# cgbur/llama2.zig

Measured on AMD Instinct MI355X. Metric: tokens/s (argmax, -t 0), higher is better.
Workload: dtype f32; 1 GPU; llama2-7b shape, fp32 llama2.c-v0 checkpoint (dim 4096, hidden 11008, L 32, H 32, kv 32, V 32000, S 2048), greedy from BOS, seeded synthetic weights; parallelism=1 GPU

## Files before the change

### llama2.zig_amd/binding.py

```python
from __future__ import annotations

import ctypes as C
import os
import re

import numpy as np

_HERE = os.path.dirname(os.path.abspath(__file__))
PRODUCT_LIB_PATH = os.path.join(_HERE, "libllama2_hip.so")
LIB_PATH = os.environ.get("L2Z_LIB") or os.path.join(_HERE, "libllama2_hip_test.so")
HEADER_PATH = os.path.join(os.path.dirname(_HERE), "include", "llama2_hip.h")
TEST_HEADER_PATH = os.path.join(os.path.dirname(_HERE), "include", "llama2_hip_test.h")

OK, ERR_INVALID, ERR_NO_DEVICE, ERR_HIP, ERR_OOM, ERR_COMM, ERR_STATE = 0, -1, -2, -3, -4, -5, -6
COMM_ID_BYTES = 128
COMM_IPC_BYTES = 64
KINDS = ["qkv", "attn", "wo", "ffn13", "ffn2", "cls", "argmax", "gather"]


class L2ZError(RuntimeError):
    def __init__(self, code: int, msg: str):
        super().__init__(f"llama2_hip error {code}: {msg}")
        self.code = code

# ... 1277 lines not shown


def softmax(x) -> np.ndarray:
    o = np.array(x, np.float32, copy=True)
    _chk(lib().l2z_softmax(_fp(o), o.size))
    return o


def vector_dot_product(x, y) -> np.float32:
    x, y = _f32(x), _f32(y)
    o = np.zeros(1, np.float32)
    _chk(lib().l2z_vector_dot_product(_fp(o), _fp(x), _fp(y), x.size))
    return o[0]


def vector_weighted_sum_rows(xout_len: int, rows, row_stride: int, weights) -> np.ndarray:
    rows, weights = _f32(rows), _f32(weights)
    o = np.empty(xout_len, np.float32)
    _chk(lib().l2z_vector_weighted_sum_rows(_fp(o), xout_len, _fp(rows), rows.size, row_stride,
                                            _fp(weights), weights.size))
    return o


ATTN_FORMS = {"auto": 0, "fast256": 1, "fast1024": 2, "split": 3, "generic": 4}


def attention_decode(q, kcache, vcache, pos: int, n_heads: int, n_kv_heads: int, head_size: int,
                     seq_len: int, form: str = "auto", nch: int = 0) -> np.ndarray:
    q, kcache, vcache = _f32(q), _f32(kcache), _f32(vcache)
    assert q.size == n_heads * head_size and kcache.size == seq_len * n_kv_heads * head_size
    out = np.empty(n_heads * head_size, np.float32)
    _chk(lib().l2z_attention_decode(ATTN_FORMS[form], nch, _fp(out), _fp(q), _fp(kcache), _fp(vcache),
                                    pos, n_heads, n_kv_heads, head_size, seq_len))
    return out


def q8_quantize(x, gs: int):
    x = _f32(x).reshape(-1)
    q = np.empty(x.size, np.int8)
    s = np.empty(x.size // gs, np.float32)
    _chk(lib().l2z_q8_quantize(_fp(x), x.size, gs, q.ctypes.data_as(C.POINTER(C.c_int8)), _fp(s)))
    return q, s


def q8_matmul(xq, xs, wq, ws, gs: int) -> np.ndarray:
    wq = np.ascontiguousarray(wq, dtype=np.int8)
    d, n = wq.shape
# ... 105 lines not shown
```

### llama2.zig_amd/csrc/attention.hip

```cpp
#include "kernel_common.h"

namespace l2z {
namespace {

constexpr int kAttnUB = 4;

template <bool VEC>
__device__ __forceinline__ void attn_scores(const float *qs, const float *__restrict__ kbase,
                                            int kv_stride, int head_size, int T, float div,
                                            float *att)
{
    const AttnGeom ge = attn_geom(head_size, VEC);
    const int g = threadIdx.x / ge.TPR, c0 = threadIdx.x % ge.TPR;
    for (int t0 = g; t0 < T; t0 += ge.G * kAttnUB) {
        float p[kAttnUB];
#pragma unroll
        for (int i = 0; i < kAttnUB; i++) p[i] = 0.0f;
        for (int c = c0; c < ge.E; c += ge.TPR) {
            if (VEC) {
                v4f kv[kAttnUB];
#pragma unroll
                for (int i = 0; i < kAttnUB; i++) {
                    int t = t0 + ge.G * i;
                    t = t < T ? t : T - 1;
// ... 64 lines not shown
            for (int t0 = g; t0 < T; t0 += ge.G * kAttnUB) {
                float vv[kAttnUB], w[kAttnUB];
#pragma unroll
                for (int i = 0; i < kAttnUB; i++) {
                    const int t = t0 + ge.G * i;
                    const int tc = t < T ? t : T - 1;
                    vv[i] = vbase[(size_t)tc * (size_t)kv_stride + c];
                    w[i] = t < T ? att[tc] : 0.0f;
                }
#pragma unroll
                for (int i = 0; i < kAttnUB; i++) acc = fmaf(vv[i], w[i], acc);
            }
            part[(size_t)g * head_size + c] = acc;
        }
    }
    __syncthreads();
    for (int i = threadIdx.x; i < head_size; i += blockDim.x) {
        float s = part[i];
        for (int gg = 1; gg < ge.G; gg++) s += part[(size_t)gg * head_size + i];
        out[i] = s;
    }
}

template <bool WT = false>
__device__ __forceinline__ void reduce_partials(const float *part, int G, int hs, float *out,
                                                const P2pArgs *push = nullptr, int push_e = 0,
                                                size_t push_idx0 = 0)
{
    int R = 1;
    while (R * 2 <= G && R * 2 * hs <= (int)blockDim.x && R < 16) R <<= 1;
    const int i = threadIdx.x / R, r = threadIdx.x % R;
    float s = 0.0f;
    if (i < hs)
        for (int gg = r; gg < G; gg += R) s += part[(size_t)gg * hs + i];
    s = lanes_sum(s, R);
    if (i < hs && r == 0) {
        if constexpr (WT) {
            __hip_atomic_store(out + i, s, __ATOMIC_RELAXED, __HIP_MEMORY_SCOPE_AGENT);
        } else {
            out[i] = s;
            if (push) p2p_ll_push(push, push_e, push_idx0 + (size_t)i, s);
        }
    }
}

constexpr int kFastUB = 8;
constexpr int kAttnFastBlock = 1024;

struct AttnLane {
    int g, c0, cc, G, TPR;
    size_t stride;
};

template <bool NT>
__device__ __forceinline__ void attn_load_round(const float *base, const AttnLane &ln, int t0, int bound, v4f (&r)[kFastUB])
{
#pragma unroll
    for (int i = 0; i < kFastUB; i++) {
        int t = t0 + ln.G * i;
        t = t < bound ? t : bound - 1;
        const v4f *p = (const v4f *)(base + (size_t)t * ln.stride) + ln.cc;
        if constexpr (NT) r[i] = ldg_nt(p);
        else r[i] = *p;
    }
}

template <bool NT>
__device__ __forceinline__ void attn_score_rounds(const float *kbase, const AttnLane &ln, v4f qv, v4f (&kr)[kFastUB], int T,
                                                  float div, float *att)
{
    const v4f zero = {0.f, 0.f, 0.f, 0.f};
    for (int t0 = ln.g;;) {
#pragma unroll
        for (int i = 0; i < kFastUB; i++) {
            float p = hsum4(fma4(qv, kr[i], zero));
            p = lanes_sum(p, ln.TPR);
            const int t = t0 + ln.G * i;
            if (ln.c0 == 0 && t < T) att[t] = p / div;
        }
        t0 += ln.G * kFastUB;
        if (t0 >= T) break;
        attn_load_round<NT>(kbase, ln, t0, T, kr);
    }
}

template <bool NT>
__device__ __forceinline__ v4f attn_wsum_rounds(const float *vbase, const AttnLane &ln, v4f (&vr)[kFastUB], int T, const float *w_)
{
    v4f acc = {0.f, 0.f, 0.f, 0.f};
    for (int t0 = ln.g;;) {
#pragma unroll
        for (int i = 0; i < kFastUB; i++) {
            const int t = t0 + ln.G * i;
            const float w = t < T ? w_[t] : 0.0f;
            acc.x = fmaf(vr[i].x, w, acc.x);
            acc.y = fmaf(vr[i].y, w, acc.y);
            acc.z = fmaf(vr[i].z, w, acc.z);
            acc.w = fmaf(vr[i].w, w, acc.w);
        }
        t0 += ln.G * kFastUB;
        if (t0 >= T) break;
        attn_load_round<NT>(vbase, ln, t0, T, vr);
    }
    return acc;
}

__device__ __forceinline__ AttnLane attn_lane(const AttnGeom &ge, size_t stride)
{
    AttnLane ln;
    ln.g = threadIdx.x / ge.TPR;
    ln.c0 = threadIdx.x % ge.TPR;
    ln.cc = ln.c0 < ge.E ? ln.c0 : 0;
    ln.G = ge.G;
    ln.TPR = ge.TPR;
    ln.stride = stride;
    return ln;
}

template <int NT, bool SPEC>
__global__ __launch_bounds__(NT) void attention_fast_kernel(const AttnArgs a)
{
    extern __shared__ __attribute__((aligned(16))) float lds[];
// ... 5 lines not shown
    const int h = blockIdx.x;
    const int kvh = h / a.kv_mul;
    const float *kbase = a.kcache + (size_t)kvh * a.kv_head;
    const float *vbase = a.vcache + (size_t)kvh * a.kv_head;
    const AttnLane ln = attn_lane(ge, (size_t)a.kv_row);
    const bool active = ln.c0 < ge.E;
    const v4f zero = {0.f, 0.f, 0.f, 0.f};

    const int T = *a.pos_ptr + 1;
    const int lim = SPEC ? a.seq_len : T;
    const v4f qv = active ? ((const v4f *)(a.q + (size_t)h * hs))[ln.cc] : zero;
    v4f kr[kFastUB], vr[kFastUB];
    attn_load_round<false>(kbase, ln, ln.g, lim, kr);
    attn_load_round<false>(vbase, ln, ln.g, lim, vr);
    attn_score_rounds<false>(kbase, ln, qv, kr, T, sqrtf((float)hs), att);
    __syncthreads();
    wave_softmax(att, prob, T);
    const v4f acc = attn_wsum_rounds<false>(vbase, ln, vr, T, prob);
    if (active) ((v4f *)(part + (size_t)ln.g * hs))[ln.cc] = acc;
    __syncthreads();
    reduce_partials(part, ge.G, hs, a.xb + (size_t)h * hs, a.push,
                    a.push ? a.push_ctl[kCtlEpoch] + a.push_gi : 0,
                    a.push ? (size_t)a.push->rank * a.push->count + (size_t)h * hs : 0);
}

__host__ __device__ inline int attn_split_per(int T, int nch) { return (((T + nch - 1) / nch) + 1) & ~1; }

__device__ __forceinline__ void combine_chunks(const float *p, int nch, int hs, float *xb_h,
                                               const P2pArgs *push, int push_e, size_t push_idx0)
{
    constexpr int kMaxCh = 16;
    float mc[kMaxCh], lc[kMaxCh];
#pragma unroll
    for (int c = 0; c < kMaxCh; c++) {
        const int cc = c < nch ? c : 0;
        mc[c] = p[(size_t)cc * (hs + 4) + hs];
        lc[c] = p[(size_t)cc * (hs + 4) + hs + 1];
    }
    float M = -INFINITY;
#pragma unroll
    for (int c = 0; c < kMaxCh; c++)
        if (c < nch) M = fmaxf(M, mc[c]);
    float den = 0.0f;
#pragma unroll
    for (int c = 0; c < kMaxCh; c++) {
        mc[c] = c < nch ? expf(mc[c] - M) : 0.0f;
// ... 203 lines not shown
static bool attn_vec_shape(const AttnArgs &a)
{
    return (a.head_size % 4) == 0 && (a.kv_row % 4) == 0 && (a.kv_head % 4) == 0 && aligned16(a.q) && aligned16(a.kcache) &&
           aligned16(a.vcache);
}
static bool attn_fast_shape(const AttnArgs &a) { return attn_vec_shape(a) && a.head_size <= 256; }

bool attention_push_supported(const AttnArgs &a) { return attn_fast_shape(a); }

bool attention_split_supported(const AttnArgs &a) { return attn_fast_shape(a); }

hipError_t launch_attention_split(const AttnArgs &a, int n_heads_local, int nch, float *part,
                                  int *arrivals, hipStream_t st, bool small)
{
    const int nt = small ? kBlock : kAttnFastBlock;
    const AttnGeom ge = attn_geom(a.head_size, true, nt);
    const int max_local = attn_split_per(a.seq_len, nch);
    const size_t lds = (size_t)(2 * ((max_local + 3) & ~3) + ge.G * a.head_size) * sizeof(float);
    const dim3 grid(n_heads_local * nch);
    return small ? launch_lds(attention_split_kernel<kBlock>, grid, dim3(kBlock), lds, st, a, nch, part, arrivals)
                 : launch_lds(attention_split_kernel<kAttnFastBlock>, grid, dim3(kAttnFastBlock), lds, st, a, nch, part, arrivals);
}

hipError_t launch_attention(const AttnArgs &a, int n_heads_local, hipStream_t st, int form)
{
    const bool vec = attn_vec_shape(a);
    const dim3 grid(n_heads_local);
    if (attn_fast_shape(a) && form != 4) {
        const int forced = form == 1 ? kBlock : form == 2 ? kAttnFastBlock : 0;
        const int nt = forced ? forced : (a.seq_len > 512 ? kAttnFastBlock : kBlock);
        const AttnGeom gf = attn_geom(a.head_size, true, nt);
        const size_t lds_fast = (size_t)(2 * ((a.seq_len + 3) & ~3) + gf.G * a.head_size) * sizeof(float);
        return nt == kAttnFastBlock ? launch_lds(attention_fast_kernel<kAttnFastBlock, false>, grid, dim3(kAttnFastBlock), lds_fast, st, a)
                                    : launch_lds(attention_fast_kernel<kBlock, true>, grid, dim3(kBlock), lds_fast, st, a);
    }
    const size_t lds = attention_lds_bytes(a.head_size, a.seq_len, vec);
    return vec ? launch_lds(attention_kernel<true>, grid, dim3(kBlock), lds, st, a)
               : launch_lds(attention_kernel<false>, grid, dim3(kBlock), lds, st, a);
}

hipError_t launch_dot(float *out, const float *x, const float *y, int n, hipStream_t st)
{
    const bool vec = (n % 4) == 0 && aligned16(x) && aligned16(y);
    if (vec)
        hipLaunchKernelGGL((dot_kernel<true>), dim3(1), dim3(kBlock), 0, st, out, x, y, n);
    else
// ... 36 lines not shown
```

### llama2.zig_amd/csrc/forward.cpp

```cpp
#include <algorithm>
#include <cmath>
#include <cstdlib>
#include <cstring>
#include <mutex>

#include "batch_host.h"
#include "kind_rows.h"
#include "l2z_state.h"

namespace l2z {

struct Prof {
    std::vector<hipEvent_t> ev;
    std::vector<int> kind;
};

#define L2Z_LAUNCH(kind_id, expr)                                                         \
    do {                                                                                  \
        hipEvent_t _a = nullptr, _b = nullptr;                                            \
        if (prof) {                                                                       \
            L2Z_HIP(hipEventCreate(&_a));                                                 \
            L2Z_HIP(hipEventCreate(&_b));                                                 \
            L2Z_HIP(hipEventRecord(_a, st));                                              \
        }                                                                                 \
// ... 161 lines not shown
            a.out0 = s->q; a.out1 = kc; a.out2 = vc;
            a.rows0 = sh.dim_loc; a.rows1 = sh.kvd_loc; a.rows2 = sh.kvd_loc;
            a.pos_stride1 = sh.hs; a.pos_stride2 = sh.hs; a.kv_head_stride = kvh_stride;
            a.n = c.dim; a.rms_w = w->rms_att + (size_t)l * dim;
            x_in(a, s->x, gi, sh.dim_loc);
            a.pos_ptr = s->d_pos; a.rope = s->rope; a.head_size = sh.hs; a.rope_segs = 2;
            L2Z_LAUNCH(KIND_QKV, row_launch(KIND_QKV, l, a, PRO_RMS, EPI_ROPE));
        }
        if (!fused && want() && kind(KIND_ATTN)) {
            AttnArgs a = {};
            a.q = s->q; a.kcache = kc; a.vcache = vc; a.xb = s->xb + sh.dim0;
            a.pos_ptr = s->d_pos; a.head_size = sh.hs; a.kv_row = sh.hs; a.kv_head = kvh_stride;
            a.kv_mul = c.n_heads / c.n_kv_heads; a.seq_len = c.seq_len;
            a.tl_seq = s->tl_attn_seq++;
            if (!sb && can_push && attention_push_supported(a)) {
                a.push = s->d_push + 0;
                a.push_ctl = ctl;
                a.push_gi = comm_gi(lc, gi + 1);
                pushed = true;
            }
            if (split && s->attn_nch > 1 && attention_split_supported(a))
                L2Z_LAUNCH(KIND_ATTN, launch_attention_split(a, sh.heads_loc, s->attn_nch,
                                                             s->d_attn_part, s->d_attn_cnt, st, variant == ATTN_SPLIT_S));
            else
                L2Z_LAUNCH(KIND_ATTN, launch_attention(a, sh.heads_loc, st, variant == ATTN_SHORT ? 1 : 0));
        }
        if (!sb) L2Z_TRY(gather(s->xb, sh.dim_loc));
        if (want() && kind(KIND_WO)) {
            MatvecArgs a = {};
            int epi = EPI_RESID;
            if (sb) {
                col_shard(a, s->xb + sh.dim0, sh.dimc_pad, &epi);
            } else {
                a.out0 = s->x + sh.dim0; a.resid = s->x + sh.dim0;
                a.rows0 = sh.dim_loc; a.n = c.dim;
                x_in(a, s->xb, gi, sh.dim_loc);
                push_to(a, 1);
            }
            L2Z_LAUNCH(KIND_WO, row_launch(KIND_WO, l, a, PRO_NONE, epi));
        }
        if (sb) L2Z_TRY(reduce());
        else L2Z_TRY(gather(s->x, sh.dim_loc));
        if (want() && kind(KIND_FFN13)) {
            MatvecArgs a = {};
            a.out0 = sb ? s->hb : s->hb + sh.hid0;
            a.rows0 = sh.hid_loc; a.rows1 = sh.hid_loc; a.n = c.dim;
// ... 52 lines not shown
            a.xchg = s->d_push + 3;
            a.xchg_gi = comm_gi(lc, n_g);
            a.epoch_ctl = lc->d_ctl;
            a.epoch_add = lc->solo ? 0 : n_g;
        }
        L2Z_LAUNCH(KIND_ARGMAX, launch_argmax(a, st));
    }
    if (step == STEP_SAMPLE && want() && kind(KIND_ARGMAX)) {
        L2Z_CHECK(sh.world == 1 && s->d_smp_ctl != nullptr && s->d_smp_scratch != nullptr, L2Z_ERR_STATE,
                  "sampled step on a runstate l2z_sample_run has not prepared");
        SampleStepArgs a = {};
        a.logits = s->logits; a.vocab = c.vocab_size; a.seq_len = c.seq_len;
        a.params = (const SampleStepParams *)s->d_smp_ctl; a.coins = s->d_smp_ctl + 2; a.scratch = s->d_smp_scratch;
        a.token_ptr = s->d_token; a.pos_ptr = s->d_pos; a.prompt = s->d_prompt; a.n_prompt_ptr = s->d_n_prompt;
        a.out_tokens = s->d_out_tokens; a.tok_emb = w->tok_emb; a.emb_q8 = w->q8_emb(); a.x = s->x; a.dim = c.dim;
        L2Z_LAUNCH(KIND_ARGMAX, launch_sample_step(a, st));
    }
    return L2Z_OK;
}

int attn_variant(const l2z_runstate *s, int pos)
{
    if (s->attn_nch > 1 && pos >= s->attn_split_pos) return pos < s->attn_split_wide_pos ? ATTN_SPLIT_S : ATTN_SPLIT;
    return pos < s->attn_short_pos ? ATTN_SHORT : ATTN_HEAD;
}

int build_graph(l2z_runstate *s, const l2z_weights *w, StepKind step, int variant,
                hipGraphExec_t *out)
{
    hipGraph_t graph = nullptr;
    L2Z_HIP(hipStreamBeginCapture(s->stream, hipStreamCaptureModeThreadLocal));
    int rc = enqueue_forward(s, w, step, nullptr, -1, variant);
    hipError_t e = hipStreamEndCapture(s->stream, &graph);
    if (rc != L2Z_OK) {
        if (graph) (void)hipGraphDestroy(graph);
        return rc;
    }
    L2Z_HIP(e);
    e = hipGraphInstantiate(out, graph, nullptr, nullptr, 0);
    (void)hipGraphDestroy(graph);
    L2Z_HIP(e);
    return L2Z_OK;
}

void drop_graphs(l2z_runstate *s)
{
    for (int v = 0; v < ATTN_VARIANTS; v++) {
        if (s->g_forward[v]) { (void)hipGraphExecDestroy(s->g_forward[v]); s->g_forward[v] = nullptr; }
        if (s->g_step[v]) { (void)hipGraphExecDestroy(s->g_step[v]); s->g_step[v] = nullptr; }
        if (s->g_sample[v]) { (void)hipGraphExecDestroy(s->g_sample[v]); s->g_sample[v] = nullptr; }
    }
    s->graph_w_uid = 0;
}

hipGraphExec_t *graph_slot(l2z_runstate *s, StepKind step, int variant)
{
    return step == STEP_SAMPLE ? &s->g_sample[variant] : step == STEP_GREEDY ? &s->g_step[variant] : &s->g_forward[variant];
}

int ensure_graph(l2z_runstate *s, const l2z_weights *w, int variant, StepKind step)
{
    if (!s->use_graphs) return L2Z_OK;
    int rc = L2Z_OK;
    if (s->graph_w_uid != w->uid) {
        drop_graphs(s);
        s->graph_w_uid = w->uid;
        const int edges[] = {0, s->attn_short_pos, s->attn_split_pos, s->attn_split_wide_pos, s->cfg.seq_len};
        bool reach[ATTN_VARIANTS] = {};
        for (int e : edges)
            for (int p = e - 1; p <= e; p++)
                if (p >= 0 && p < s->cfg.seq_len) reach[attn_variant(s, p)] = true;
        for (int v = 0; v < ATTN_VARIANTS && rc == L2Z_OK; v++) {
            if (!reach[v]) continue;
            rc = build_graph(s, w, STEP_NONE, v, &s->g_forward[v]);
            if (rc == L2Z_OK) rc = build_graph(s, w, STEP_GREEDY, v, &s->g_step[v]);
        }
    }
    hipGraphExec_t *slot = graph_slot(s, step, variant);
    if (rc == L2Z_OK && *slot) return L2Z_OK;
    if (rc != L2Z_OK || build_graph(s, w, step, variant, slot) != L2Z_OK) {
        fprintf(stderr, "llama2_hip: hipGraph capture failed (%s); launching eagerly\n", l2z_last_error());
        drop_graphs(s);
        s->use_graphs = false;
        (void)hipGetLastError();
    }
    return L2Z_OK;
}

int run_forward(l2z_runstate *s, const l2z_weights *w, StepKind step, int pos)
{
// ... 330 lines not shown
```

### llama2.zig_amd/csrc/hooks.cpp

```cpp
#include <algorithm>
#include <cmath>
#include <cstdlib>
#include <cstring>
#include <mutex>

#include "l2z_state.h"

using namespace l2z;

namespace {
struct DevBuf {
    float *p = nullptr;
    ~DevBuf() { if (p) (void)hipFree(p); }
    int alloc(size_t n) { L2Z_HIP(hipMalloc(&p, (n ? n : 1) * sizeof(float))); return L2Z_OK; }
    int up(const float *h, size_t n) { L2Z_HIP(hipMemcpy(p, h, n * sizeof(float), hipMemcpyHostToDevice)); return L2Z_OK; }
    int down(float *h, size_t n) { L2Z_HIP(hipMemcpy(h, p, n * sizeof(float), hipMemcpyDeviceToHost)); return L2Z_OK; }
};
}

extern "C" int l2z_matmul_fused(int N, float *const *outs, const float *x, const float *const *ws,
                                size_t n, size_t d)
{
    L2Z_CHECK(N >= 1 && N <= kMaxSeg && outs && x && ws && n > 0 && d > 0, L2Z_ERR_INVALID,
              "l2z_matmul_fused: bad arguments");
// ... 122 lines not shown
    const size_t dim = (size_t)n_heads * head_size, kvd = (size_t)n_kv_heads * head_size;
    DevBuf dq, dk, dv, dout;
    L2Z_TRY(dq.alloc(n_queries * dim)); L2Z_TRY(dk.alloc(seq_len * kvd)); L2Z_TRY(dv.alloc(seq_len * kvd));
    L2Z_TRY(dout.alloc(n_queries * dim));
    const std::vector<float> hk = to_head_major(kcache, seq_len, n_kv_heads, head_size),
                             hv = to_head_major(vcache, seq_len, n_kv_heads, head_size);
    L2Z_TRY(dq.up(q, n_queries * dim)); L2Z_TRY(dk.up(hk.data(), seq_len * kvd)); L2Z_TRY(dv.up(hv.data(), seq_len * kvd));
    const hipError_t e = launch_prefill_attention(dq.p, (int)dim, dk.p, dv.p, dout.p, (int)dim, pos0, n_queries, n_heads,
                                                  head_size, head_size, (size_t)seq_len * head_size, n_heads / n_kv_heads,
                                                  seq_len, nullptr, n_heads, form);
    L2Z_HIP(e);
    L2Z_HIP(hipDeviceSynchronize());
    L2Z_TRY(dout.down(out, n_queries * dim));
    return L2Z_OK;
}

extern "C" int l2z_attention_decode(int form, int nch, float *out, const float *q, const float *kcache,
                                    const float *vcache, int pos, int n_heads, int n_kv_heads,
                                    int head_size, int seq_len)
{
    L2Z_CHECK(out && q && kcache && vcache && n_heads > 0 && n_kv_heads > 0 && head_size > 0 &&
                  n_heads % n_kv_heads == 0 && seq_len > 0 && pos >= 0 && pos < seq_len,
              L2Z_ERR_INVALID, "l2z_attention_decode: bad arguments");
    L2Z_CHECK(form >= 0 && form <= 4, L2Z_ERR_INVALID, "l2z_attention_decode: form %d", form);
    L2Z_TRY(ensure_device(current_device_for(nullptr)));
    const size_t dim = (size_t)n_heads * head_size, kvd = (size_t)n_kv_heads * head_size;
    const size_t kvn = (size_t)seq_len * kvd;
    DevBuf dq, dk, dv, dout, dpart;
    int *dpos = nullptr, *dcnt = nullptr;
    L2Z_TRY(dq.alloc(dim)); L2Z_TRY(dk.alloc(kvn)); L2Z_TRY(dv.alloc(kvn)); L2Z_TRY(dout.alloc(dim));
    const std::vector<float> hk = to_head_major(kcache, seq_len, n_kv_heads, head_size),
                             hv = to_head_major(vcache, seq_len, n_kv_heads, head_size);
    L2Z_TRY(dq.up(q, dim)); L2Z_TRY(dk.up(hk.data(), kvn)); L2Z_TRY(dv.up(hv.data(), kvn));
    AttnArgs a = {};
    a.q = dq.p; a.kcache = dk.p; a.vcache = dv.p; a.xb = dout.p;
    a.head_size = head_size; a.kv_row = head_size; a.kv_head = (size_t)seq_len * head_size;
    a.kv_mul = n_heads / n_kv_heads; a.seq_len = seq_len;
    const bool fast_ok = attention_split_supported(a);
    L2Z_CHECK(form == 0 || form == 4 || fast_ok, L2Z_ERR_INVALID,
              "l2z_attention_decode: form %d needs head_size %% 4 == 0 and <= 256", form);
    const size_t att_lds = attention_lds_bytes(head_size, seq_len, fast_ok);
    L2Z_CHECK(att_lds <= 160 * 1024, L2Z_ERR_INVALID, "l2z_attention_decode: seq_len too long for LDS");
    hipError_t e = hipMalloc(&dpos, sizeof(int));
    if (e == hipSuccess) e = hipMemcpy(dpos, &pos, sizeof(int), hipMemcpyHostToDevice);
    a.pos_ptr = dpos;
    int use_nch = 0;
    if (e == hipSuccess && (form == 3 || (form == 0 && fast_ok && pos >= 256 && seq_len > 256))) {
        use_nch = nch > 0 ? nch : attention_split_chunks(n_heads, g_cus);
        if (use_nch > 16) use_nch = 16;
        if (use_nch < 2) use_nch = form == 3 ? 2 : 0;
    }
    if (e == hipSuccess && use_nch > 1) {
        int rc = dpart.alloc(attention_split_part_floats(n_heads, head_size, use_nch));
        if (rc != L2Z_OK) { (void)hipFree(dpos); return rc; }
        e = hipMalloc(&dcnt, (size_t)n_heads * sizeof(int));
        if (e == hipSuccess) e = hipMemset(dcnt, 0, (size_t)n_heads * sizeof(int));
        const bool small = pos < attention_split_wide_pos(seq_len);
        if (e == hipSuccess) e = launch_attention_split(a, n_heads, use_nch, dpart.p, dcnt, nullptr, small);
        if (e == hipSuccess) e = launch_attention_split(a, n_heads, use_nch, dpart.p, dcnt, nullptr, small);
    } else if (e == hipSuccess) {
        const int auto_form = pos < attention_short_pos(head_size, seq_len) ? 1 : 0;
        e = launch_attention(a, n_heads, nullptr, form == 3 || form == 0 ? auto_form : form);
    }
    if (e == hipSuccess) e = hipDeviceSynchronize();
    (void)hipFree(dpos);
    if (dcnt) (void)hipFree(dcnt);
    L2Z_HIP(e);
    return dout.down(out, dim);
}

extern "C" int l2z_option_set(const char *env_name, long long value)
{
    L2Z_CHECK(env_name != nullptr && tunables_set(env_name, value), L2Z_ERR_INVALID,
              "l2z_option_set: unknown option '%s'", env_name ? env_name : "(null)");
    return L2Z_OK;
}

extern "C" int l2z_shard_plan(const l2z_config *config, int rank, int world, int *out, int cap)
{
    L2Z_CHECK(config != nullptr && out != nullptr && cap >= 10 && world >= 1 && rank >= 0 && rank < world, L2Z_ERR_INVALID,
              "l2z_shard_plan: bad arguments");
    l2z_comm c;
    c.rank = rank; c.world = world; c.device = 0; c.nccl = nullptr;
    Shard sh;
    L2Z_TRY(make_shard(*config, &c, &sh));
// ... 229 lines not shown
```

### llama2.zig_amd/csrc/l2z_internal.h

```cpp
#pragma once

#include <hip/hip_runtime.h>

#include <cstdarg>
#include <cstdint>
#include <cstdio>
#include <string>
#include <vector>

#include "../../include/llama2_hip.h"
#include "../../include/llama2_hip_test.h"

namespace l2z {

struct P2pArgs;

struct LLIn {
    const unsigned long long *slots;
    unsigned slot_floats;
    unsigned count;
    int gi;
    int *ctl;
    int *h_err;
    long long timeout_ticks;
// ... 150 lines not shown
bool fused_qkv_attn_supported(int dim, int n_heads, int n_kv_heads, int seq_len, int n_cus);
hipError_t launch_fused_qkv_attn(const FusedQkvAttnArgs &a, int n_heads, hipStream_t st);

hipError_t launch_pk_stats(const float *m, size_t count, uint32_t *stats, hipStream_t st);
hipError_t launch_pk_pack(const float *m, int rows, int n, int e_base, uint32_t *pk, hipStream_t st);
hipError_t launch_pk_unpack(const uint32_t *pk, int rows, int n, int e_base, float *out, hipStream_t st);
hipError_t launch_pk28_count(const float *m, int rows, int n, int e_base, uint32_t *max_esc, hipStream_t st);
hipError_t launch_pk28_pack(const float *m, int rows, int n, int e_base, uint32_t *pk, uint32_t *rec, hipStream_t st);
hipError_t launch_pk28_unpack(const uint32_t *pk, const uint32_t *rec, int rows, int n, int e_base, float *out, hipStream_t st);
hipError_t launch_matvec(const MatvecArgs &a, int pro, int epi, int max_blocks_per_cu, int n_cus,
                         hipStream_t st, int *out_grid = nullptr, bool *pushed = nullptr);
bool attention_push_supported(const AttnArgs &a);
int matvec_max_grid(int n_cus);
bool matvec_vector_width(int n);
hipError_t launch_stream_read(const float *p, size_t n_floats, float *out, int n_cus, hipStream_t st);
hipError_t launch_attention(const AttnArgs &a, int n_heads_local, hipStream_t st, int form = 0);
int attention_short_pos(int head_size, int seq_len);
int attention_split_chunks(int n_heads_local, int n_cus);
size_t attention_split_part_floats(int n_heads_local, int head_size, int nch);
bool attention_split_supported(const AttnArgs &a);
hipError_t launch_attention_split(const AttnArgs &a, int n_heads_local, int nch, float *part,
                                  int *arrivals, hipStream_t st, bool small = false);
int attention_split_wide_pos(int seq_len);
hipError_t launch_argmax(const ArgmaxArgs &a, hipStream_t st);
hipError_t launch_set_state(int token, int pos, int *token_ptr, int *pos_ptr, const float *tok_emb,
                            float *x, int dim, hipStream_t st);
hipError_t launch_rmsnorm(float *o, const float *x, const float *w, int n, hipStream_t st);
hipError_t launch_softmax(float *x, int n, hipStream_t st);
hipError_t launch_probs(float *probs, const float *logits, int n, float temperature, hipStream_t st);
hipError_t launch_dot(float *out, const float *x, const float *y, int n, hipStream_t st);
hipError_t launch_weighted_sum_rows(float *xout, int xout_len, const float *rows, int row_stride,
                                    const float *weights, int n_weights, hipStream_t st);
hipError_t launch_synth_fill(float *dst, uint64_t base_idx, uint64_t count, uint64_t seed,
                             float scale, float bias, hipStream_t st, uint64_t row_len = 0, uint64_t row_pitch = 0,
                             uint64_t idx_pitch = 0);
hipError_t launch_sum_parts(float *out, const float *const *parts, int n_parts, int n, hipStream_t st);
hipError_t launch_copy_rows(float *dst, size_t dpitch, const float *src, size_t rows, size_t cols, hipStream_t st);
size_t attention_lds_bytes(int head_size, int seq_len, bool vec);

struct SplitKWs {
    float *part;
    int *cnt;
    size_t part_floats;
    int cnt_ints;
    void *x3;
    size_t x3_bytes;
// ... 144 lines not shown
```

### llama2.zig_amd/csrc/l2z_state.h

```cpp
#pragma once
#include <cstdint>
#include <vector>

#include "kv_pages.h"
#include "l2z_comm.h"
#include "l2z_internal.h"
#include "tunables.h"

namespace l2z {

struct BatchScratch;
struct WideScratch;

struct Shard {
    int rank = 0, world = 1;
    int hs = 0;
    int dim0 = 0, dim_loc = 0;
    int kvd_loc = 0;
    int heads_loc = 0;
    int hid0 = 0, hid_loc = 0;
    int v0 = 0, v_loc = 0;
    bool scheme_b = false;
    int dimc_pad = 0, hidc_pad = 0;
};
// ... 103 lines not shown
    float *pf_part = nullptr;
    int *pf_tokens = nullptr;
    l2z::DeferredSum pf_pending = {nullptr, 1, 128, 1, false};
    l2z::PlanesReady pf_planes_att = l2z::PLANES_SPLIT, pf_planes_h1 = l2z::PLANES_SPLIT;
    l2z::SplitKWs pf_sk = {nullptr, nullptr, 0, 0, nullptr, 0, nullptr, 0};
    int pf_cap = 0;
    void *sc_ws = nullptr, *sc_seq = nullptr;
    size_t sc_ws_bytes = 0;
    int sc_cap = 0, sc_slab_n = 0;
    int sc_slab_force = 0;
    float *d_probs = nullptr;
    float *h_stage = nullptr;
    float *d_smp_ctl = nullptr, *h_smp_ctl = nullptr, *d_smp_scratch = nullptr;
    float *d_part_val = nullptr;
    int *d_part_idx = nullptr;
    int n_part = 0;
    int n_part_step = 0, n_part_fwd = 0;
    float *d_attn_part = nullptr;
    int *d_attn_cnt = nullptr;
    int attn_nch = 0;
    int attn_split_pos = 0;
    int attn_short_pos = 0;
    int attn_split_wide_pos = 0;
    uint64_t graph_w_uid = 0;
    hipGraphExec_t g_forward[4] = {nullptr, nullptr, nullptr, nullptr}, g_step[4] = {nullptr, nullptr, nullptr, nullptr};
    hipGraphExec_t g_sample[4] = {nullptr, nullptr, nullptr, nullptr};
    bool use_graphs = true;
    int host_pos = 0;
    bool done = false;
    std::vector<int32_t> h_prompt;
    l2z::P2pArgs *d_push = nullptr;
    int n_gathers = 0;
    bool ll_consume = false;
    bool xchg_steps = false;
    bool logits_partial = false;
    bool fused_qkv_attn = false;
    int max_blocks = 0;
    bool packed_w = true;
    int packed_kinds = -1;
    int tl_attn_seq = 0;
    l2z::BatchScratch *bt = nullptr;
    float *rg_k = nullptr, *rg_v = nullptr;
    void *rg_tab = nullptr;
    int rg_cap = 0;
    l2z::WideScratch *wd = nullptr;
};

namespace l2z {

struct Prof;
int check_pair(const l2z_config *config, const l2z_runstate *s, const l2z_weights *w, bool paged_ok = false,
               bool q8_ok = false);
enum { ATTN_SHORT = 0, ATTN_HEAD = 1, ATTN_SPLIT_S = 2, ATTN_SPLIT = 3, ATTN_VARIANTS = 4 };
enum StepKind { STEP_NONE = 0, STEP_GREEDY = 1, STEP_SAMPLE = 2 };
int enqueue_forward(l2z_runstate *s, const l2z_weights *w, StepKind step, Prof *prof, int only_stage,
                    int variant, int only_kind = -1);
int attn_variant(const l2z_runstate *s, int pos);
int run_forward(l2z_runstate *s, const l2z_weights *w, StepKind step, int pos);
int ensure_logits(l2z_runstate *s);
void drop_graphs(l2z_runstate *s);

constexpr int kPrefillMinPrompt = L2Z_PREFILL_MIN_PROMPT;
bool prefill_enabled();
bool prefill_usable(const l2z_runstate *s);
bool prefill_shard_takes_the_unsharded_kernels(const l2z_config &c, const Shard &sh);
int prefill_check(const l2z_config *config, const l2z_runstate *s);
struct ScoreCall;
int prefill_tokens(l2z_runstate *s, const l2z_weights *w, const int32_t *tokens, int n_tokens, int pos0,
                   const ScoreCall *score = nullptr);

int prefill_scratch(l2z_runstate *s, int need);
int prefill_ragged_chunk(l2z_runstate *s, const l2z_weights *w, const int32_t *tokens, int P, const RaggedChunk &rg);
int prefill_last_logits(l2z_runstate *s, const l2z_weights *w);
int prefill_rows_logits(l2z_runstate *s, const l2z_weights *w, int P, float *out, int ldo, const int *rows = nullptr);
int ragged_alloc(l2z_runstate *s, int need);

// ... 16 lines not shown
```

### llama2.zig_amd/csrc/runstate.cpp

```cpp
#include <algorithm>
#include <cmath>
#include <cstdlib>
#include <cstring>
#include <mutex>
#include <vector>

#include "l2z_state.h"

using namespace l2z;

static int runstate_make(const l2z_config *config, const l2z_comm *comm, l2z_kvpool *pool, l2z_runstate **out)
{
    L2Z_CHECK(config != nullptr && out != nullptr, L2Z_ERR_INVALID, "runstate_init: null argument");
    const int dev = current_device_for(comm);
    L2Z_TRY(ensure_device(dev));
    Shard sh;
    L2Z_TRY(make_shard(*config, comm, &sh));
    const l2z_config &c = *config;
    const size_t att_lds = attention_lds_bytes(sh.hs, c.seq_len, sh.hs % 4 == 0 && sh.kvd_loc % 4 == 0);
    L2Z_CHECK(att_lds <= 160 * 1024, L2Z_ERR_INVALID,
              "seq_len %d needs %zu bytes of LDS for attention scores (max 163840)", c.seq_len,
              att_lds);
    const int n_max = c.dim > c.hidden_dim ? c.dim : c.hidden_dim;
    L2Z_CHECK(matvec_lds_bytes(n_max) <= 160 * 1024, L2Z_ERR_INVALID,
// ... 45 lines not shown
        alloc((void **)&s->d_pages, s->pg.pages.size() * 4);
        if (e == hipSuccess) e = hipHostMalloc((void **)&s->h_pages, s->pg.pages.size() * 4, hipHostMallocDefault);
        s->pages_dirty = true;
    }
    alloc((void **)&s->rope, (size_t)c.seq_len * (sh.hs / 2) * sizeof(float2));
    alloc((void **)&s->d_token, 4);
    alloc((void **)&s->d_pos, 4);
    alloc((void **)&s->d_n_prompt, 4);
    alloc((void **)&s->d_argmax, 4);
    alloc((void **)&s->d_prompt, (size_t)c.seq_len * 4);
    alloc((void **)&s->d_out_tokens, (size_t)c.seq_len * 4);
    alloc((void **)&s->d_part_val, (size_t)matvec_max_grid(g_cus) * 4);
    alloc((void **)&s->d_part_idx, (size_t)matvec_max_grid(g_cus) * 4);
    {
        const int mode = tn.attn_split;
        int nch = mode > 0 ? mode : attention_split_chunks(c.n_heads, g_cus);
        if (nch > 16) nch = 16;
        s->attn_split_pos = mode > 0 ? 0 : 256;
        if (tn.attn_split_pos >= 0) s->attn_split_pos = tn.attn_split_pos;
        if (mode == 0 || c.seq_len <= s->attn_split_pos) nch = 0;
        s->attn_split_wide_pos = attention_split_wide_pos(c.seq_len);
        s->attn_short_pos = attention_short_pos(sh.hs, c.seq_len);
        if (nch > 1 && s->attn_short_pos > s->attn_split_pos) s->attn_short_pos = s->attn_split_pos;
        if (nch > 1) {
            s->attn_nch = nch;
            alloc((void **)&s->d_attn_part, attention_split_part_floats(sh.heads_loc, sh.hs, nch) * 4);
            alloc((void **)&s->d_attn_cnt, (size_t)sh.heads_loc * 4);
        }
    }
    if (comm_uses_p2p(comm) && e == hipSuccess) {
        AttnArgs aa = {};
        aa.q = s->q; aa.kcache = s->key_cache; aa.vcache = s->value_cache;
        aa.head_size = sh.hs; aa.kv_row = sh.hs; aa.kv_head = (size_t)c.seq_len * sh.hs;
        const bool want_consume = tn.p2p_consume >= 0 ? tn.p2p_consume != 0 : (sh.world <= 2 || c.dim < 4096);
        s->ll_consume = !sh.scheme_b && want_consume && matvec_vector_width(c.dim) &&
                        matvec_vector_width(c.hidden_dim) && attention_push_supported(aa);
        P2pArgs t[4];
        comm_p2p_args(comm, s->xb, (size_t)sh.dim_loc, s->ll_consume, &t[0]);
        comm_p2p_args(comm, sh.scheme_b ? s->part : s->x, sh.scheme_b ? (size_t)c.dim : (size_t)sh.dim_loc, s->ll_consume, &t[1]);
        comm_p2p_args(comm, s->hb, (size_t)sh.hid_loc, s->ll_consume, &t[2]);
        comm_p2p_args(comm, s->logits, (size_t)sh.v_loc, false, &t[3]);
        alloc((void **)&s->d_push, sizeof t);
        if (e == hipSuccess) e = hipMemcpy(s->d_push, t, sizeof t, hipMemcpyHostToDevice);
        s->xchg_steps = tn.argmax_xchg != 0 && matvec_vector_width(c.dim) && sh.v_loc >= 2 && comm->slot_floats >= 2 * (size_t)sh.world;
    }
    if (e != hipSuccess) {
// ... 225 lines not shown
```

### llama2.zig_amd/csrc/tunables.cpp

```cpp
#include "tunables.h"

#include <cstdlib>
#include <cstring>

namespace l2z {
namespace {

void env_int(const char *name, int *v)
{
    if (const char *e = getenv(name))
        if (*e) *v = atoi(e);
}

Tunables read_env()
{
    Tunables t;
    env_int("L2Z_GRID_CAP", &t.grid_cap);
    env_int("L2Z_ATTN_SPLIT", &t.attn_split);
    env_int("L2Z_ATTN_SPLIT_POS", &t.attn_split_pos);
    env_int("L2Z_FUSE_SMALL", &t.fuse_small);
    env_int("L2Z_SCHEME_B", &t.scheme_b);
    env_int("L2Z_NO_GRAPH", &t.no_graph);
    if (const char *e = getenv("L2Z_COMM")) t.prefer_rccl = strcmp(e, "rccl") == 0;
    env_int("L2Z_ARGMAX_XCHG", &t.argmax_xchg);
    env_int("L2Z_P2P_CONSUME", &t.p2p_consume);
    if (const char *e = getenv("L2Z_P2P_TIMEOUT_S"))
        if (*e) t.p2p_timeout_s = atoll(e);
    env_int("L2Z_P2P_BULK_MB", &t.p2p_bulk_mb);
    env_int("L2Z_PREFILL", &t.prefill);
    env_int("L2Z_PF_CHUNK", &t.pf_chunk);
    env_int("L2Z_PF_PANEL", &t.pf_panel);
    env_int("L2Z_PF_PANEL_MAX", &t.pf_panel_max);
    env_int("L2Z_PF_X3", &t.pf_x3);
    env_int("L2Z_PF_X3_STREAM_MIN", &t.pf_x3_stream_min);
    env_int("L2Z_PF_FUSE_PLANES", &t.pf_fuse_planes);
    env_int("L2Z_PACKED_W", &t.packed_w);
    env_int("L2Z_PACKED_KINDS", &t.packed_kinds);
    env_int("L2Z_PACKED_BITS", &t.packed_bits);
    env_int("L2Z_PACKED28_KINDS", &t.packed28_kinds);
    return t;
}

// ... 8 lines not shown
}

const Tunables &tunables() { return mutable_tunables(); }

int prefill_chunk_tokens()
{
    int n = tunables().pf_chunk > 0 ? tunables().pf_chunk : 1024;
    if (n < 16) n = 16;
    if (n > 2048) n = 2048;
    return n;
}

int prefill_next_chunk(int remaining)
{
    if (tunables().pf_chunk > 0) return remaining < prefill_chunk_tokens() ? remaining : prefill_chunk_tokens();
    return remaining >= 1024 ? 1024 : remaining < 512 ? remaining : 512;
}

bool tunables_set(const char *name, long long v)
{
    Tunables &t = mutable_tunables();
    struct { const char *n; int *p; } ints[] = {
        {"L2Z_GRID_CAP", &t.grid_cap}, {"L2Z_ATTN_SPLIT", &t.attn_split}, {"L2Z_ATTN_SPLIT_POS", &t.attn_split_pos},
        {"L2Z_FUSE_SMALL", &t.fuse_small}, {"L2Z_NO_GRAPH", &t.no_graph}, {"L2Z_SCHEME_B", &t.scheme_b},
        {"L2Z_COMM_RCCL", &t.prefer_rccl}, {"L2Z_ARGMAX_XCHG", &t.argmax_xchg}, {"L2Z_P2P_CONSUME", &t.p2p_consume},
        {"L2Z_P2P_BULK_MB", &t.p2p_bulk_mb}, {"L2Z_PREFILL", &t.prefill}, {"L2Z_PF_CHUNK", &t.pf_chunk},
        {"L2Z_PF_PANEL", &t.pf_panel}, {"L2Z_PF_PANEL_MAX", &t.pf_panel_max},
        {"L2Z_PF_X3", &t.pf_x3}, {"L2Z_PF_X3_STREAM_MIN", &t.pf_x3_stream_min},
        {"L2Z_PF_FUSE_PLANES", &t.pf_fuse_planes}, {"L2Z_PACKED_W", &t.packed_w},
        {"L2Z_PACKED_KINDS", &t.packed_kinds}, {"L2Z_PACKED_BITS", &t.packed_bits},
        {"L2Z_PACKED28_KINDS", &t.packed28_kinds}};
    for (auto &e : ints)
        if (strcmp(e.n, name) == 0) {
            *e.p = (int)v;
            return true;
        }
    if (strcmp(name, "L2Z_P2P_TIMEOUT_S") == 0) {
        t.p2p_timeout_s = v;
        return true;
    }
    return false;
}

}
```

### llama2.zig_amd/csrc/tunables.h

```cpp
#pragma once

namespace l2z {

struct Tunables {
    int grid_cap = 0;
    int attn_split = -1;
    int attn_split_pos = -1;
    int fuse_small = 1;
    int no_graph = 0;
    int prefer_rccl = 0;
    int p2p_consume = -1;
    int argmax_xchg = 1;
    long long p2p_timeout_s = 20;
    int scheme_b = 0;
    int p2p_bulk_mb = -1;
    int prefill = 1;
    int pf_chunk = 0;
    int pf_panel = 1;
    int pf_x3 = 1;
    int pf_x3_stream_min = 33;
    int pf_fuse_planes = 1;
    int packed_w = 1;
    int packed_kinds = -1;
    int packed_bits = 28;
    int packed28_kinds = 40;
    int pf_panel_max = -1;

    static constexpr int row_blocks = 2;
    static constexpr int max_blocks_per_cu = 8;
    static constexpr int p2p_push = 1;
    static constexpr int reduce_block = 128;
    static constexpr int pf_skinny_max = 64;
};

const Tunables &tunables();
int prefill_chunk_tokens();
int prefill_next_chunk(int remaining);
bool tunables_set(const char *env_name, long long value);

}
```

Baseline: 246.7 tokens/s.

## Add head-sliced attention decode kernel that splits each head's value sum across blocks

Adds an attention kernel that launches several blocks per head, each recomputing the full score row and softmax but summing only a slice of the head dimension over the value cache. It is used by default with 4 slices for positions from 64 up to the short-attention threshold on single-GPU runs. The aim is more blocks in flight while the context is short, to better fill the GPU and overlap K/V loads. The cost is redundant QK score and softmax work in each slice, plus an extra graph variant.

```diff
diff --git a/llama2.zig_amd/binding.py b/llama2.zig_amd/binding.py
--- a/llama2.zig_amd/binding.py
+++ b/llama2.zig_amd/binding.py
@@ -1323,7 +1323,7 @@
     return o
 
 
-ATTN_FORMS = {"auto": 0, "fast256": 1, "fast1024": 2, "split": 3, "generic": 4}
+ATTN_FORMS = {"auto": 0, "fast256": 1, "fast1024": 2, "split": 3, "generic": 4, "sliced256": 5, "sliced1024": 6}
 
 
 def attention_decode(q, kcache, vcache, pos: int, n_heads: int, n_kv_heads: int, head_size: int,
diff --git a/llama2.zig_amd/csrc/attention.hip b/llama2.zig_amd/csrc/attention.hip
--- a/llama2.zig_amd/csrc/attention.hip
+++ b/llama2.zig_amd/csrc/attention.hip
@@ -110,13 +110,18 @@
     }
 }
 
+__host__ __device__ inline int attn_reduce_lanes(int G, int hs, int nt)
+{
+    int R = 1;
+    while (R * 2 <= G && R * 2 * hs <= nt && R < 16) R <<= 1;
+    return R;
+}
+
 template <bool WT = false>
-__device__ __forceinline__ void reduce_partials(const float *part, int G, int hs, float *out,
-                                                const P2pArgs *push = nullptr, int push_e = 0,
-                                                size_t push_idx0 = 0)
-{
-    int R = 1;
-    while (R * 2 <= G && R * 2 * hs <= (int)blockDim.x && R < 16) R <<= 1;
+__device__ __forceinline__ void reduce_partials_r(const float *part, int G, int hs, int R, float *out,
+                                                  const P2pArgs *push = nullptr, int push_e = 0,
+                                                  size_t push_idx0 = 0)
+{
     const int i = threadIdx.x / R, r = threadIdx.x % R;
     float s = 0.0f;
     if (i < hs)
@@ -132,6 +137,14 @@
     }
 }
 
+template <bool WT = false>
+__device__ __forceinline__ void reduce_partials(const float *part, int G, int hs, float *out,
+                                                const P2pArgs *push = nullptr, int push_e = 0,
+                                                size_t push_idx0 = 0)
+{
+    reduce_partials_r<WT>(part, G, hs, attn_reduce_lanes(G, hs, (int)blockDim.x), out, push, push_e, push_idx0);
+}
+
 constexpr int kFastUB = 8;
 constexpr int kAttnFastBlock = 1024;
 
@@ -153,39 +166,50 @@
     }
 }
 
+__device__ __forceinline__ void attn_score_round(const AttnLane &ln, v4f qv, const v4f (&kr)[kFastUB], int t0, int T, float div,
+                                                 float *att)
+{
+    const v4f zero = {0.f, 0.f, 0.f, 0.f};
+#pragma unroll
+    for (int i = 0; i < kFastUB; i++) {
+        float p = hsum4(fma4(qv, kr[i], zero));
+        p = lanes_sum(p, ln.TPR);
+        const int t = t0 + ln.G * i;
+        if (ln.c0 == 0 && t < T) att[t] = p / div;
+    }
+}
+
 template <bool NT>
 __device__ __forceinline__ void attn_score_rounds(const float *kbase, const AttnLane &ln, v4f qv, v4f (&kr)[kFastUB], int T,
                                                   float div, float *att)
 {
-    const v4f zero = {0.f, 0.f, 0.f, 0.f};
     for (int t0 = ln.g;;) {
-#pragma unroll
-        for (int i = 0; i < kFastUB; i++) {
-            float p = hsum4(fma4(qv, kr[i], zero));
-            p = lanes_sum(p, ln.TPR);
-            const int t = t0 + ln.G * i;
-            if (ln.c0 == 0 && t < T) att[t] = p / div;
-        }
+        attn_score_round(ln, qv, kr, t0, T, div, att);
         t0 += ln.G * kFastUB;
         if (t0 >= T) break;
         attn_load_round<NT>(kbase, ln, t0, T, kr);
     }
 }
 
+__device__ __forceinline__ void attn_wsum_round(const AttnLane &ln, const v4f (&vr)[kFastUB], int t0, int T, const float *w_, v4f &acc)
+{
+#pragma unroll
+    for (int i = 0; i < kFastUB; i++) {
+        const int t = t0 + ln.G * i;
+        const float w = t < T ? w_[t] : 0.0f;
+        acc.x = fmaf(vr[i].x, w, acc.x);
+        acc.y = fmaf(vr[i].y, w, acc.y);
+        acc.z = fmaf(vr[i].z, w, acc.z);
+        acc.w = fmaf(vr[i].w, w, acc.w);
+    }
+}
+
 template <bool NT>
 __device__ __forceinline__ v4f attn_wsum_rounds(const float *vbase, const AttnLane &ln, v4f (&vr)[kFastUB], int T, const float *w_)
 {
     v4f acc = {0.f, 0.f, 0.f, 0.f};
     for (int t0 = ln.g;;) {
-#pragma unroll
-        for (int i = 0; i < kFastUB; i++) {
-            const int t = t0 + ln.G * i;
-            const float w = t < T ? w_[t] : 0.0f;
-            acc.x = fmaf(vr[i].x, w, acc.x);
-            acc.y = fmaf(vr[i].y, w, acc.y);
-            acc.z = fmaf(vr[i].z, w, acc.z);
-            acc.w = fmaf(vr[i].w, w, acc.w);
-        }
+        attn_wsum_round(ln, vr, t0, T, w_, acc);
         t0 += ln.G * kFastUB;
         if (t0 >= T) break;
         attn_load_round<NT>(vbase, ln, t0, T, vr);
@@ -237,6 +261,88 @@
     reduce_partials(part, ge.G, hs, a.xb + (size_t)h * hs, a.push,
                     a.push ? a.push_ctl[kCtlEpoch] + a.push_gi : 0,
                     a.push ? (size_t)a.push->rank * a.push->count + (size_t)h * hs : 0);
+}
+
+constexpr int kAttnSlicedBlock = 512;
+
+template <bool SPEC>
+__global__ __launch_bounds__(kAttnSlicedBlock) void attention_sliced_kernel(const AttnArgs a, int ns, int short_pos)
+{
+    extern __shared__ __attribute__((aligned(16))) float lds[];
+    const int hs = a.head_size, hss = hs / ns;
+    const AttnGeom gk = attn_geom(hs, true, kAttnSlicedBlock);
+    float *att = lds;
+    float *prob = att + ((a.seq_len + 3) & ~3);
+    float *part = prob + ((a.seq_len + 3) & ~3);
+    const int nh = gridDim.x / ns;
+    const int h = blockIdx.x % nh, sl = blockIdx.x / nh;
+    const int kvh = h / a.kv_mul;
+    const float *kbase = a.kcache + (size_t)kvh * a.kv_head;
+    const float *vbase = a.vcache + (size_t)kvh * a.kv_head;
+    const AttnLane lk = attn_lane(gk, (size_t)a.kv_row);
+    const v4f zero = {0.f, 0.f, 0.f, 0.f};
+    const int kstep = gk.G * kFastUB;
+
+    const v4f qv = lk.c0 < gk.E ? ((const v4f *)(a.q + (size_t)h * hs))[lk.cc] : zero;
+    v4f kr0[kFastUB], kr1[kFastUB], vr0[kFastUB], vr1[kFastUB];
+    if constexpr (SPEC) attn_load_round<false>(kbase, lk, lk.g, a.seq_len, kr0);
+    const int T = *a.pos_ptr + 1;
+    if constexpr (!SPEC) attn_load_round<false>(kbase, lk, lk.g, T, kr0);
+    const bool kpre = kstep < T;
+    if (kpre) attn_load_round<false>(kbase, lk, lk.g + kstep, T, kr1);
+
+    const int nte = T - 1 < short_pos ? kBlock : kAttnFastBlock;
+    const AttnGeom ge = attn_geom(hs, true, nte);
+    const int R = attn_reduce_lanes(ge.G, hs, nte);
+    const int es = ge.E / ns;
+    int tprs = 1;
+    while (tprs < es) tprs <<= 1;
+    AttnLane lv;
+    lv.g = threadIdx.x / tprs;
+    lv.c0 = threadIdx.x % tprs;
+    lv.cc = sl * es + (lv.c0 < es ? lv.c0 : 0);
+    lv.G = ge.G;
+    lv.TPR = tprs;
+    lv.stride = (size_t)a.kv_row;
+    const bool vlane = lv.g < ge.G;
+    const int vstep = ge.G * kFastUB;
+    const bool vpre = vstep < T;
+    if (vlane) {
+        attn_load_round<false>(vbase, lv, lv.g, T, vr0);
+        if (vpre) attn_load_round<false>(vbase, lv, lv.g + vstep, T, vr1);
+    }
+
+    {
+        const float div = sqrtf((float)hs);
+        int t0 = lk.g;
+        attn_score_round(lk, qv, kr0, t0, T, div, att);
+        t0 += kstep;
+        if (t0 < T) {
+            attn_score_round(lk, qv, kr1, t0, T, div, att);
+            for (t0 += kstep; t0 < T; t0 += kstep) {
+                attn_load_round<false>(kbase, lk, t0, T, kr0);
+                attn_score_round(lk, qv, kr0, t0, T, div, att);
+            }
+        }
+    }
+    __syncthreads();
+    wave_softmax(att, prob, T);
+    if (vlane) {
+        v4f acc = zero;
+        int t0 = lv.g;
+        attn_wsum_round(lv, vr0, t0, T, prob, acc);
+        t0 += vstep;
+        if (t0 < T) {
+            attn_wsum_round(lv, vr1, t0, T, prob, acc);
+            for (t0 += vstep; t0 < T; t0 += vstep) {
+                attn_load_round<false>(vbase, lv, t0, T, vr0);
+                attn_wsum_round(lv, vr0, t0, T, prob, acc);
+            }
+        }
+        if (lv.c0 < es) ((v4f *)(part + (size_t)lv.g * hss))[lv.c0] = acc;
+    }
+    __syncthreads();
+    reduce_partials_r(part, ge.G, hss, R, a.xb + (size_t)h * hs + (size_t)sl * hss);
 }
 
 __host__ __device__ inline int attn_split_per(int T, int nch) { return (((T + nch - 1) / nch) + 1) & ~1; }
@@ -486,6 +592,28 @@
                  : launch_lds(attention_split_kernel<kAttnFastBlock>, grid, dim3(kAttnFastBlock), lds, st, a, nch, part, arrivals);
 }
 
+int attention_slices(int head_size, int seq_len, int knob)
+{
+    const int ns = knob < 0 ? Tunables::attn_slices_default : (knob & 15);
+    if (ns < 2 || seq_len <= 512 || head_size != 128 || ((head_size / 4) % ns) != 0) return 0;
+    return ns;
+}
+
+bool attention_sliced_supported(const AttnArgs &a, int ns)
+{
+    return attn_fast_shape(a) && a.push == nullptr && ns >= 2 && ns <= 16 && ((a.head_size / 4) % ns) == 0;
+}
+
+hipError_t launch_attention_sliced(const AttnArgs &a, int n_heads_local, int ns, int short_pos, bool spec, hipStream_t st)
+{
+    if (!attention_sliced_supported(a, ns)) return hipErrorInvalidValue;
+    const AttnGeom gw = attn_geom(a.head_size, true, kAttnFastBlock);
+    const size_t lds = (size_t)(2 * ((a.seq_len + 3) & ~3) + gw.G * (a.head_size / ns)) * sizeof(float);
+    const dim3 grid(n_heads_local * ns);
+    return spec ? launch_lds(attention_sliced_kernel<true>, grid, dim3(kAttnSlicedBlock), lds, st, a, ns, short_pos)
+                : launch_lds(attention_sliced_kernel<false>, grid, dim3(kAttnSlicedBlock), lds, st, a, ns, short_pos);
+}
+
 hipError_t launch_attention(const AttnArgs &a, int n_heads_local, hipStream_t st, int form)
 {
     const bool vec = attn_vec_shape(a);
diff --git a/llama2.zig_amd/csrc/forward.cpp b/llama2.zig_amd/csrc/forward.cpp
--- a/llama2.zig_amd/csrc/forward.cpp
+++ b/llama2.zig_amd/csrc/forward.cpp
@@ -207,6 +207,8 @@
             if (split && s->attn_nch > 1 && attention_split_supported(a))
                 L2Z_LAUNCH(KIND_ATTN, launch_attention_split(a, sh.heads_loc, s->attn_nch,
                                                              s->d_attn_part, s->d_attn_cnt, st, variant == ATTN_SPLIT_S));
+            else if (variant == ATTN_SLICED)
+                L2Z_LAUNCH(KIND_ATTN, launch_attention_sliced(a, sh.heads_loc, s->attn_slices, s->attn_short_pos, s->attn_sliced_spec, st));
             else
                 L2Z_LAUNCH(KIND_ATTN, launch_attention(a, sh.heads_loc, st, variant == ATTN_SHORT ? 1 : 0));
         }
@@ -305,6 +307,7 @@
 int attn_variant(const l2z_runstate *s, int pos)
 {
     if (s->attn_nch > 1 && pos >= s->attn_split_pos) return pos < s->attn_split_wide_pos ? ATTN_SPLIT_S : ATTN_SPLIT;
+    if (s->attn_slices > 1 && pos >= s->attn_sliced_pos && pos < s->attn_sliced_end) return ATTN_SLICED;
     return pos < s->attn_short_pos ? ATTN_SHORT : ATTN_HEAD;
 }
 
@@ -348,7 +351,7 @@
     if (s->graph_w_uid != w->uid) {
         drop_graphs(s);
         s->graph_w_uid = w->uid;
-        const int edges[] = {0, s->attn_short_pos, s->attn_split_pos, s->attn_split_wide_pos, s->cfg.seq_len};
+        const int edges[] = {0, s->attn_short_pos, s->attn_sliced_pos, s->attn_sliced_end, s->attn_split_pos, s->attn_split_wide_pos, s->cfg.seq_len};
         bool reach[ATTN_VARIANTS] = {};
         for (int e : edges)
             for (int p = e - 1; p <= e; p++)
diff --git a/llama2.zig_amd/csrc/hooks.cpp b/llama2.zig_amd/csrc/hooks.cpp
--- a/llama2.zig_amd/csrc/hooks.cpp
+++ b/llama2.zig_amd/csrc/hooks.cpp
@@ -168,7 +168,7 @@
     L2Z_CHECK(out && q && kcache && vcache && n_heads > 0 && n_kv_heads > 0 && head_size > 0 &&
                   n_heads % n_kv_heads == 0 && seq_len > 0 && pos >= 0 && pos < seq_len,
               L2Z_ERR_INVALID, "l2z_attention_decode: bad arguments");
-    L2Z_CHECK(form >= 0 && form <= 4, L2Z_ERR_INVALID, "l2z_attention_decode: form %d", form);
+    L2Z_CHECK(form >= 0 && form <= 6, L2Z_ERR_INVALID, "l2z_attention_decode: form %d", form);
     L2Z_TRY(ensure_device(current_device_for(nullptr)));
     const size_t dim = (size_t)n_heads * head_size, kvd = (size_t)n_kv_heads * head_size;
     const size_t kvn = (size_t)seq_len * kvd;
@@ -185,6 +185,9 @@
     const bool fast_ok = attention_split_supported(a);
     L2Z_CHECK(form == 0 || form == 4 || fast_ok, L2Z_ERR_INVALID,
               "l2z_attention_decode: form %d needs head_size %% 4 == 0 and <= 256", form);
+    const bool sliced = form == 5 || form == 6;
+    L2Z_CHECK(!sliced || attention_sliced_supported(a, nch & 15), L2Z_ERR_INVALID,
+              "l2z_attention_decode: %d slices need (head_size / 4) %% slices == 0, 2 <= slices <= 15", nch & 15);
     const size_t att_lds = attention_lds_bytes(head_size, seq_len, fast_ok);
     L2Z_CHECK(att_lds <= 160 * 1024, L2Z_ERR_INVALID, "l2z_attention_decode: seq_len too long for LDS");
     hipError_t e = hipMalloc(&dpos, sizeof(int));
@@ -204,9 +207,15 @@
         const bool small = pos < attention_split_wide_pos(seq_len);
         if (e == hipSuccess) e = launch_attention_split(a, n_heads, use_nch, dpart.p, dcnt, nullptr, small);
         if (e == hipSuccess) e = launch_attention_split(a, n_heads, use_nch, dpart.p, dcnt, nullptr, small);
+    } else if (e == hipSuccess && sliced) {
+        e = launch_attention_sliced(a, n_heads, nch & 15, form == 5 ? seq_len : 0, (nch & 16) != 0, nullptr);
     } else if (e == hipSuccess) {
-        const int auto_form = pos < attention_short_pos(head_size, seq_len) ? 1 : 0;
-        e = launch_attention(a, n_heads, nullptr, form == 3 || form == 0 ? auto_form : form);
+        const int short_pos = attention_short_pos(head_size, seq_len);
+        const int knob = tunables().attn_slices, ns = attention_slices(head_size, seq_len, knob);
+        if (form == 0 && ns > 1 && pos >= Tunables::attn_sliced_pos && pos < short_pos && attention_sliced_supported(a, ns))
+            e = launch_attention_sliced(a, n_heads, ns, short_pos, knob > 0 && (knob & 16) != 0, nullptr);
+        else
+            e = launch_attention(a, n_heads, nullptr, form == 3 || form == 0 ? (pos < short_pos ? 1 : 0) : form);
     }
     if (e == hipSuccess) e = hipDeviceSynchronize();
     (void)hipFree(dpos);
diff --git a/llama2.zig_amd/csrc/l2z_internal.h b/llama2.zig_amd/csrc/l2z_internal.h
--- a/llama2.zig_amd/csrc/l2z_internal.h
+++ b/llama2.zig_amd/csrc/l2z_internal.h
@@ -196,6 +196,9 @@
 hipError_t launch_attention_split(const AttnArgs &a, int n_heads_local, int nch, float *part,
                                   int *arrivals, hipStream_t st, bool small = false);
 int attention_split_wide_pos(int seq_len);
+int attention_slices(int head_size, int seq_len, int knob);
+bool attention_sliced_supported(const AttnArgs &a, int ns);
+hipError_t launch_attention_sliced(const AttnArgs &a, int n_heads_local, int ns, int short_pos, bool spec, hipStream_t st);
 hipError_t launch_argmax(const ArgmaxArgs &a, hipStream_t st);
 hipError_t launch_set_state(int token, int pos, int *token_ptr, int *pos_ptr, const float *tok_emb,
                             float *x, int dim, hipStream_t st);
diff --git a/llama2.zig_amd/csrc/l2z_state.h b/llama2.zig_amd/csrc/l2z_state.h
--- a/llama2.zig_amd/csrc/l2z_state.h
+++ b/llama2.zig_amd/csrc/l2z_state.h
@@ -149,9 +149,12 @@
     int attn_split_pos = 0;
     int attn_short_pos = 0;
     int attn_split_wide_pos = 0;
+    int attn_slices = 0;
+    int attn_sliced_pos = 0, attn_sliced_end = 0;
+    bool attn_sliced_spec = false;
     uint64_t graph_w_uid = 0;
-    hipGraphExec_t g_forward[4] = {nullptr, nullptr, nullptr, nullptr}, g_step[4] = {nullptr, nullptr, nullptr, nullptr};
-    hipGraphExec_t g_sample[4] = {nullptr, nullptr, nullptr, nullptr};
+    hipGraphExec_t g_forward[5] = {nullptr, nullptr, nullptr, nullptr, nullptr}, g_step[5] = {nullptr, nullptr, nullptr, nullptr, nullptr};
+    hipGraphExec_t g_sample[5] = {nullptr, nullptr, nullptr, nullptr, nullptr};
     bool use_graphs = true;
     int host_pos = 0;
     bool done = false;
@@ -178,7 +181,7 @@
 struct Prof;
 int check_pair(const l2z_config *config, const l2z_runstate *s, const l2z_weights *w, bool paged_ok = false,
                bool q8_ok = false);
-enum { ATTN_SHORT = 0, ATTN_HEAD = 1, ATTN_SPLIT_S = 2, ATTN_SPLIT = 3, ATTN_VARIANTS = 4 };
+enum { ATTN_SHORT = 0, ATTN_HEAD = 1, ATTN_SPLIT_S = 2, ATTN_SPLIT = 3, ATTN_SLICED = 4, ATTN_VARIANTS = 5 };
 enum StepKind { STEP_NONE = 0, STEP_GREEDY = 1, STEP_SAMPLE = 2 };
 int enqueue_forward(l2z_runstate *s, const l2z_weights *w, StepKind step, Prof *prof, int only_stage,
                     int variant, int only_kind = -1);
diff --git a/llama2.zig_amd/csrc/runstate.cpp b/llama2.zig_amd/csrc/runstate.cpp
--- a/llama2.zig_amd/csrc/runstate.cpp
+++ b/llama2.zig_amd/csrc/runstate.cpp
@@ -91,6 +91,14 @@
         s->attn_split_wide_pos = attention_split_wide_pos(c.seq_len);
         s->attn_short_pos = attention_short_pos(sh.hs, c.seq_len);
         if (nch > 1 && s->attn_short_pos > s->attn_split_pos) s->attn_short_pos = s->attn_split_pos;
+        if (sh.world == 1 && !s->fused_qkv_attn) {
+            s->attn_slices = attention_slices(sh.hs, c.seq_len, tn.attn_slices);
+            s->attn_sliced_spec = tn.attn_slices > 0 && (tn.attn_slices & 16) != 0;
+            const bool whole = tn.attn_slices > 0 && (tn.attn_slices & 32) != 0;
+            s->attn_sliced_pos = whole ? 0 : Tunables::attn_sliced_pos;
+            s->attn_sliced_end = whole ? (nch > 1 ? s->attn_split_pos : 256) : s->attn_short_pos;
+            if (s->attn_sliced_end <= s->attn_sliced_pos) s->attn_slices = 0;
+        }
         if (nch > 1) {
             s->attn_nch = nch;
             alloc((void **)&s->d_attn_part, attention_split_part_floats(sh.heads_loc, sh.hs, nch) * 4);
diff --git a/llama2.zig_amd/csrc/tunables.cpp b/llama2.zig_amd/csrc/tunables.cpp
--- a/llama2.zig_amd/csrc/tunables.cpp
+++ b/llama2.zig_amd/csrc/tunables.cpp
@@ -18,6 +18,7 @@
     env_int("L2Z_GRID_CAP", &t.grid_cap);
     env_int("L2Z_ATTN_SPLIT", &t.attn_split);
     env_int("L2Z_ATTN_SPLIT_POS", &t.attn_split_pos);
+    env_int("L2Z_ATTN_SLICES", &t.attn_slices);
     env_int("L2Z_FUSE_SMALL", &t.fuse_small);
     env_int("L2Z_SCHEME_B", &t.scheme_b);
     env_int("L2Z_NO_GRAPH", &t.no_graph);
@@ -72,7 +73,7 @@
     Tunables &t = mutable_tunables();
     struct { const char *n; int *p; } ints[] = {
         {"L2Z_GRID_CAP", &t.grid_cap}, {"L2Z_ATTN_SPLIT", &t.attn_split}, {"L2Z_ATTN_SPLIT_POS", &t.attn_split_pos},
-        {"L2Z_FUSE_SMALL", &t.fuse_small}, {"L2Z_NO_GRAPH", &t.no_graph}, {"L2Z_SCHEME_B", &t.scheme_b},
+        {"L2Z_ATTN_SLICES", &t.attn_slices}, {"L2Z_FUSE_SMALL", &t.fuse_small}, {"L2Z_NO_GRAPH", &t.no_graph}, {"L2Z_SCHEME_B", &t.scheme_b},
         {"L2Z_COMM_RCCL", &t.prefer_rccl}, {"L2Z_ARGMAX_XCHG", &t.argmax_xchg}, {"L2Z_P2P_CONSUME", &t.p2p_consume},
         {"L2Z_P2P_BULK_MB", &t.p2p_bulk_mb}, {"L2Z_PREFILL", &t.prefill}, {"L2Z_PF_CHUNK", &t.pf_chunk},
         {"L2Z_PF_PANEL", &t.pf_panel}, {"L2Z_PF_PANEL_MAX", &t.pf_panel_max},
diff --git a/llama2.zig_amd/csrc/tunables.h b/llama2.zig_amd/csrc/tunables.h
--- a/llama2.zig_amd/csrc/tunables.h
+++ b/llama2.zig_amd/csrc/tunables.h
@@ -6,6 +6,7 @@
     int grid_cap = 0;
     int attn_split = -1;
     int attn_split_pos = -1;
+    int attn_slices = -1;
     int fuse_small = 1;
     int no_graph = 0;
     int prefer_rccl = 0;
@@ -26,6 +27,8 @@
     int packed28_kinds = 40;
     int pf_panel_max = -1;
 
+    static constexpr int attn_slices_default = 4;
+    static constexpr int attn_sliced_pos = 64;
     static constexpr int row_blocks = 2;
     static constexpr int max_blocks_per_cu = 8;
     static constexpr int p2p_push = 1;
```

Result: no change. 246.7 tokens/s, median of 2 (+0.0%).
